# finlaymiller/torch-vae

Hardware: AMD Instinct MI355X
Metric: training samples/sec (VAE step: forward+ELBO+backward+AdamW), synthetic pianoroll (higher is better)
Workload: dtype bf16; 1 GPU; VanillaVAE latent_dim=16, 128x128 synthetic pianoroll, batch 256/GPU (generalised bottleneck 256*(H/16)^2); img_size=128, latent_dim=16, batch_per_gpu=256, global_batch=256, parallelism=dp1, optimizer=AdamW+OneCycle (encoder, decoder groups)

## Files before the change

### include/vae_step.h

```cpp
#ifndef VAE_STEP_H
#define VAE_STEP_H
#include <stdint.h>
#ifdef __cplusplus
extern "C" {
#endif

typedef struct vae_ctx vae_ctx;
typedef void* vae_stream_t;

#define VAE_NUM_PARAMS 40
#define VAE_NUM_BN 8
#define VAE_DTYPE_F32 0
#define VAE_DTYPE_BF16 1
#define VAE_DTYPE_F16 2

const char* vae_last_error(void);
int vae_abi_version(void);

int vae_param_layout(int img_size, int latent_dim, int generalised, int64_t* offsets ,
                     int64_t* sizes , int64_t* total);
int vae_bn_layout(int64_t* offsets , int64_t* channels , int64_t* total);

vae_ctx* vae_create(int img_size, int latent_dim, int max_batch, int dtype, int generalised);
void vae_destroy(vae_ctx* ctx);
// ... 112 lines not shown
                                 int skip_nonfinite, int64_t* step, double* norm_out, int64_t* skipped, void* scratch,
                                 int exchange, float* xhat, float* mu, float* log_var, float* z, float* out3,
                                 vae_stream_t stream);

int vae_synth_pianoroll(float* x, int batch, int img_size, uint64_t seed, vae_stream_t stream);

int vae_expand_stimuli(const void* src, int kind, float* dst, int64_t n_cells, vae_stream_t stream);

int vae_gather_rolls(const void* src, int kind, int64_t n_rolls, int h, int src_w, const int64_t* index, int64_t first,
                     const int32_t* params, uint64_t seed, uint64_t counter0, uint64_t counter_stride, int max_pitch_shift,
                     int max_time_shift, int crop_mode, float scale, float* dst, int batch, int w, vae_stream_t stream);
int vae_augment_params(int32_t* params, int batch, int src_w, int w, uint64_t seed, uint64_t counter0, uint64_t counter_stride,
                       int max_pitch_shift, int max_time_shift, int crop_mode, vae_stream_t stream);

int vae_extract_notes(const float* rolls, int64_t n, int h, int w, float onset_threshold, float sustain_threshold,
                      int min_duration, int max_gap, int32_t* events , float* peaks ,
                      int64_t capacity, int64_t* offsets , uint8_t* cleaned , vae_stream_t stream);

int vae_nearest_rolls(const uint8_t* queries , int n_queries,
                      const uint8_t* rolls   ,   int64_t n_rolls, int h, int w,
                      int max_pitch_shift, int max_time_shift, const int64_t* exclude ,
                      int k, int splits ,
                      int64_t* index , int32_t* distance ,
                      int32_t* shift , int32_t* intersection ,
                      int32_t* query_cells , vae_stream_t stream);

int vae_profile(vae_ctx* ctx, int enable);
int vae_profile_report(vae_ctx* ctx, char* buf, int64_t capacity);
int vae_profile_sequence(vae_ctx* ctx, char* buf, int64_t capacity);
int vae_profile_timeline(vae_ctx* ctx, char* buf, int64_t capacity);
int vae_debug_stamps(vae_ctx* ctx, const char* tag, int epi, long long* out);

int vae_debug_tensor(vae_ctx* ctx, int which, float* out, int64_t capacity, vae_stream_t stream);
int vae_selftest_tr16(vae_stream_t stream);
int vae_set_option(vae_ctx* ctx, const char* name, int value);
int vae_option_info(int index, const char** name, int* default_value);

#ifdef __cplusplus
}
#endif
#endif
```

### torch_vae_amd/_lib.py

```python
from __future__ import annotations

import ctypes as C
import os

_HERE = os.path.dirname(os.path.abspath(__file__))
LIB_PATH = os.environ.get("VAE_STEP_LIB") or os.path.join(_HERE, "lib", "libvae_step_gfx950.so")

NUM_PARAMS = 40
NUM_BN = 8
DTYPE_F32 = 0
DTYPE_BF16 = 1
DTYPE_F16 = 2
RECON_BCE = 0
RECON_MSE = 1
RECON_WBCE = 2
POS_WEIGHT_MAX = 1024.0
KL_PLAIN = 0
KL_FREE_BITS = 1
KL_CAPACITY = 2
KL_TC = 3
TC_MAX_BATCH = 4096
RECON_METRICS_MAX_THRESHOLDS = 8
COMM_ID_BYTES = 128
ROLLS_BYTES, ROLLS_BITS, ROLLS_F32 = 0, 1, 2
# ... 66 lines not shown
    _sig(L.vae_recon_metrics, i32, [p, p, i64, i64, f32p, i32, f32, p, p, p, p, i32, p])
    _sig(L.vae_backward, i32, [p, p, p, p, p, p, p, p, p, p, f32, i32, p])
    _sig(L.vae_backward_part, i32, [p, p, p, p, p, p, p, p, p, p, f32, i32, i32, p])
    _sig(L.vae_encode, i32, [p, p, i32, p, p, p, p, u64, i32, p, p, p, p])
    _sig(L.vae_backward_ex, i32, [p, p, p, p, p, p, p, p, p, p, f32, i32, p, p, p])
    _sig(L.vae_comm_stream, i32, [p, p, C.POINTER(C.c_void_p)])
    _sig(L.vae_comm_unique_id, i32, [p])
    _sig(L.vae_comm_init, i32, [p, i32, i32, p])
    _sig(L.vae_comm_world, i32, [p])
    _sig(L.vae_comm_destroy, i32, [p])
    _sig(L.vae_allreduce_grads, i32, [p, p, i32, i64p, i64p, i32, p])
    _sig(L.vae_broadcast_state, i32, [p, p, p, p, i32, p])
    _sig(L.vae_adamw_step, i32, [p, p, p, p, i32, i64p, i64p, f64p, f64p, f64, f64, f64, f32, i32, p])
    _sig(L.vae_grad_norm, i32, [p, i32, i64p, i64p, f32, p, p, p])
    _sig(L.vae_adamw_step_clipped, i32, [p, p, p, p, i32, i64p, i64p, f64p, f64p, f64, f64, f64, f32, f64, i32, p, p, p, p, p])
    _sig(L.vae_train_step, i32, [p, p, i32, p, p, p, p, p, p, p, u64, f32, i32, i64p, i64p, f64p, f64p, f64, f64, f64,
                                 i32, p, p, p, p, p, p])
    _sig(L.vae_train_step_fused, i32, [p, p, i32, p, p, p, p, p, p, p, u64, f32, i32, i64p, i64p, f64p, f64p, f64, f64, f64, f32,
                                       i32, i32, p, p, p, p, p, p])
    _sig(L.vae_train_step_fused_clipped, i32, [p, p, i32, p, p, p, p, p, p, p, u64, f32, i32, i64p, i64p, f64p, f64p, f64, f64, f64,
                                               f32, f64, i32, p, p, p, p, i32, p, p, p, p, p, p])
    _sig(L.vae_synth_pianoroll, i32, [p, i32, i32, u64, p])
    _sig(L.vae_expand_stimuli, i32, [p, i32, p, i64, p])
    _sig(L.vae_gather_rolls, i32, [p, i32, i64, i32, i32, p, i64, p, u64, u64, u64, i32, i32, i32, f32, p, i32, i32, p])
    _sig(L.vae_augment_params, i32, [p, i32, i32, i32, u64, u64, u64, i32, i32, i32, p])
    _sig(L.vae_extract_notes, i32, [p, i64, i32, i32, f32, f32, i32, i32, p, p, i64, p, p, p])
    _sig(L.vae_nearest_rolls, i32, [p, i32, p, i64, i32, i32, i32, i32, p, i32, i32, p, p, p, p, p, p])
    _sig(L.vae_profile, i32, [p, i32])
    _sig(L.vae_profile_report, i32, [p, C.c_char_p, i64])
    _sig(L.vae_profile_sequence, i32, [p, C.c_char_p, i64])
    _sig(L.vae_profile_timeline, i32, [p, C.c_char_p, i64])
    _sig(L.vae_debug_stamps, i32, [p, C.c_char_p, i32, p])
    _sig(L.vae_debug_tensor, i32, [p, i32, p, i64, p])
    _sig(L.vae_selftest_tr16, i32, [p])
    _sig(L.vae_set_option, i32, [p, C.c_char_p, i32])
    _sig(L.vae_option_info, i32, [i32, C.POINTER(C.c_char_p), C.POINTER(C.c_int)])
    _lib = L
    return L


EXPORTS = [
    "vae_last_error", "vae_abi_version", "vae_param_layout", "vae_bn_layout", "vae_create", "vae_destroy",
    "vae_workspace_bytes", "vae_forward", "vae_decode", "vae_pre_latents", "vae_last_eps", "vae_loss", "vae_loss_deferred", "vae_elbo_generic",
    "vae_set_recon_loss", "vae_set_recon_loss_ex", "vae_elbo_generic_ex", "vae_set_kl_objective", "vae_elbo_generic_kl", "vae_elbo_generic_w", "vae_kl_per_dim", "vae_total_correlation", "vae_last_total_correlation", "vae_log_likelihood", "vae_latent_stats",
    "vae_recon_metrics",
    "vae_backward", "vae_backward_part", "vae_encode", "vae_backward_ex", "vae_comm_stream", "vae_comm_unique_id", "vae_comm_init", "vae_comm_world",
    "vae_comm_destroy", "vae_allreduce_grads", "vae_broadcast_state", "vae_adamw_step", "vae_train_step", "vae_train_step_fused",
    "vae_grad_norm", "vae_adamw_step_clipped", "vae_train_step_fused_clipped", "vae_synth_pianoroll", "vae_expand_stimuli", "vae_profile",
    "vae_profile_report", "vae_profile_sequence", "vae_profile_timeline", "vae_debug_stamps", "vae_debug_tensor",
    "vae_selftest_tr16", "vae_set_option", "vae_option_info", "vae_gather_rolls", "vae_augment_params",
    "vae_extract_notes", "vae_nearest_rolls",
]


def check(rc: int, what: str = ""):
    if rc != 0:
        raise VaeLibError(f"{what}: {lib().vae_last_error().decode()}")


def param_layout(img_size: int, latent_dim: int, generalised: bool):
    offs = (C.c_int64 * NUM_PARAMS)()
    sizes = (C.c_int64 * NUM_PARAMS)()
    total = C.c_int64()
    rc = lib().vae_param_layout(img_size, latent_dim, int(generalised), offs, sizes, C.byref(total))
    if rc != 0:
        raise ValueError(lib().vae_last_error().decode())
    return list(offs), list(sizes), total.value


def bn_layout():
    offs = (C.c_int64 * NUM_BN)()
    ch = (C.c_int64 * NUM_BN)()
    total = C.c_int64()
    check(lib().vae_bn_layout(offs, ch, C.byref(total)), "vae_bn_layout")
    return list(offs), list(ch), total.value


def ptr(t):
    return 0 if t is None else t.data_ptr()
```

### torch_vae_amd/csrc/edge_kernels.cuh

```cuda
#pragma once
#include "common.cuh"

__device__ __forceinline__ float cg_sum(float v) {
#pragma unroll
    for (int o = 4; o < 64; o <<= 1) v += __shfl_xor(v, o, 64);
    return v;
}

template <typename T> __device__ __forceinline__ void load8(const T* p, float* o);
template <> __device__ __forceinline__ void load8<float>(const float* p, float* o) {
    f32x4 a = *reinterpret_cast<const f32x4*>(p), b = *reinterpret_cast<const f32x4*>(p + 4);
#pragma unroll
    for (int i = 0; i < 4; ++i) { o[i] = a[i]; o[4 + i] = b[i]; }
}
template <> __device__ __forceinline__ void load8<bf16>(const bf16* p, float* o) {
    bf16x8 a = *reinterpret_cast<const bf16x8*>(p);
#pragma unroll
    for (int i = 0; i < 8; ++i) o[i] = (float)a[i];
}
template <> __device__ __forceinline__ void load8<f16>(const f16* p, float* o) {
    f16x8 a = *reinterpret_cast<const f16x8*>(p);
#pragma unroll
    for (int i = 0; i < 8; ++i) o[i] = (float)a[i];
}
// ... 864 lines not shown
        const int K = d.k_is_first ? d.A : d.Bc, N = d.k_is_first ? d.Bc : d.A, pairs = d.A * d.Bc;
        for (int pr = blockIdx.x * blockDim.x + threadIdx.x; pr < pairs; pr += gridDim.x * blockDim.x) {
            const int ai = pr / d.Bc, bi = pr - ai * d.Bc;
            const int k = d.k_is_first ? ai : bi, n = d.k_is_first ? bi : ai;
            const float* sp = d.src + (size_t)pr * 9;
            float w[9];
#pragma unroll
            for (int t = 0; t < 9; ++t) w[t] = sp[t];
            const int o = ((k >> 3) * N + n) * 8 + (k & 7), plane = (K >> 3) * N * 8;
#pragma unroll
            for (int t = 0; t < 9; ++t) dst[t * plane + o] = fromfloat<T>(w[t]);
        }
        return;
    }
    for (int i = blockIdx.x * blockDim.x + threadIdx.x; i < total; i += gridDim.x * blockDim.x) {
        if (d.kind == 0) {
        } else if (d.kind == 1) {
            const int e = i & 7; const int r = i >> 3; const int n = r % d.npad; const int fp = (r / d.npad) * 8 + e;
            const int F = 256 * d.s2; const int fr = (fp & 255) * d.s2 + (fp >> 8);
            float v = 0.f;
            if (n < d.L) v = d.src[(long)n * F + fr]; else if (n < 2 * d.L) v = d.src2[(long)(n - d.L) * F + fr];
            dst[i] = fromfloat<T>(v);
        } else if (d.kind == 2) {
            const int e = i & 7; const int r = i >> 3; const int n = r % d.npad; const int fp = (r / d.npad) * 8 + e;
            const int fr = (fp & 255) * d.s2 + (fp >> 8);
            dst[i] = fromfloat<T>(n < d.L ? d.src[(long)fr * d.L + n] : 0.f);
        } else {
            const int t = i / d.A, c = i % d.A;
            reinterpret_cast<float*>(d.dst)[i] = d.src[c * 9 + t];
        }
    }
}

struct AdamGroup { long off, n; float beta1, omb1, decay; float step_size, inv_sqrt_bc2; };
struct AdamArgs {
    float* p; const float* g; float* m; float* v;
    AdamGroup grp[2]; int ngrp;
    float beta2, omb2, eps, grad_scale; int step;
};
template <bool CLIP = false>
__device__ __forceinline__ void adamw_one(float& p, float g, float& m, float& v, const AdamGroup& gr, const AdamArgs& a, float decay,
                                          float coef = 1.f) {
    g *= a.grad_scale;
    if (CLIP) g *= coef;
    p *= decay;
    m = m * gr.beta1 + gr.omb1 * g;
    v = v * a.beta2 + a.omb2 * g * g;
    const float denom = sqrtf(v) * gr.inv_sqrt_bc2 + a.eps;
    p -= gr.step_size * (m / denom);
}
template <bool CLIP = false>
__device__ __forceinline__ void adamw_range(const AdamArgs& a, const AdamGroup& gr, float coef = 1.f) {
    const float decay = gr.decay;
    const long n4 = (gr.off & 3) == 0 ? gr.n >> 2 : 0;
    for (long i = (long)blockIdx.x * blockDim.x + threadIdx.x; i < n4; i += (long)gridDim.x * blockDim.x) {
        const long k = gr.off + 4 * i;
        f32x4 p = *reinterpret_cast<const f32x4*>(a.p + k), m = *reinterpret_cast<const f32x4*>(a.m + k), v = *reinterpret_cast<const f32x4*>(a.v + k);
        const f32x4 g = *reinterpret_cast<const f32x4*>(a.g + k);
#pragma unroll
        for (int e = 0; e < 4; ++e) { float pe = p[e], me = m[e], ve = v[e]; adamw_one<CLIP>(pe, g[e], me, ve, gr, a, decay, coef); p[e] = pe; m[e] = me; v[e] = ve; }
        *reinterpret_cast<f32x4*>(a.p + k) = p; *reinterpret_cast<f32x4*>(a.m + k) = m; *reinterpret_cast<f32x4*>(a.v + k) = v;
    }
    for (long i = 4 * n4 + (long)blockIdx.x * blockDim.x + threadIdx.x; i < gr.n; i += (long)gridDim.x * blockDim.x) {
        const long k = gr.off + i;
        float pe = a.p[k], me = a.m[k], ve = a.v[k];
        adamw_one<CLIP>(pe, a.g[k], me, ve, gr, a, decay, coef);
// ... 43 lines not shown
```

### torch_vae_amd/csrc/vae_api.hip

```cpp
#include <map>
#include <mutex>
#include "vae_ctx.h"
#include "edge_kernels.cuh"
#include "loglik.cuh"
#include "grad_clip.cuh"
#include "total_corr.cuh"

static thread_local std::string g_err;
int vae_set_error(const char* what, const char* why) {
    g_err = std::string(what) + ": " + why;
    return -1;
}

extern "C" const char* vae_last_error(void) { return g_err.c_str(); }
extern "C" int vae_abi_version(void) { return 1; }

static void param_shapes(int H, int L, int gen, int64_t* sizes) {
    const int s = gen ? H / 16 : 2;
    const int64_t F = 256LL * s * s;
    const int enc_ci[4] = {1, 32, 64, 128}, enc_co[4] = {32, 64, 128, 256};
    int k = 0;
    for (int i = 0; i < 4; ++i) { sizes[k++] = 9LL * enc_ci[i] * enc_co[i]; sizes[k++] = enc_co[i]; sizes[k++] = enc_co[i]; sizes[k++] = enc_co[i]; }
    sizes[k++] = L * F; sizes[k++] = L; sizes[k++] = L * F; sizes[k++] = L; sizes[k++] = F * L; sizes[k++] = F;
    const int dec_ci[3] = {256, 128, 64}, dec_co[3] = {128, 64, 32};
// ... 48 lines not shown
    return d;
}

extern "C" void vae_destroy(vae_ctx* c) {
    if (!c) return;
    (void)vae_comm_destroy(c);
    for (void* p : c->allocs) (void)hipFree(p);
    if (c->ll_kb) (void)hipFree(c->ll_kb);
    if (c->n_side_ok) {
        for (int i = 0; i < vae_ctx::NSIDE; ++i) { (void)hipStreamSynchronize(c->side[i]); (void)hipEventDestroy(c->ev_join[i]); }
        (void)hipStreamSynchronize(c->comm);
        for (int i = 0; i < vae_ctx::NFORK; ++i) (void)hipEventDestroy(c->ev_fork[i]);
        (void)hipEventDestroy(c->ev_pack); (void)hipEventDestroy(c->ev_comm);
        if (c->ev_kl) (void)hipEventDestroy(c->ev_kl);
        for (int i = 0; i < vae_ctx::NBUCKET; ++i) (void)hipEventDestroy(c->ev_bucket[i]);
    }
    delete c;
}
extern "C" int64_t vae_workspace_bytes(const vae_ctx* c) { return c ? c->ws_bytes : 0; }

struct OptionDef { const char* name; int& (*ref)(vae_ctx&); int def; int (*norm)(int); };
static int opt_any(int v) { return v; }
static int opt_min1(int v) { return std::max(1, v); }
static int opt_fused_grid(int v) { return std::max(1, std::min(v, 512)); }
static int opt_max1024(int v) { return std::min(v, 1024); }
static int opt_max48(int v) { return std::min(v, 48); }
static int opt_fused_wgrad(int v) { return v == 1 ? 3 : v == 2 ? 1 : v == 3 ? 2 : 0; }
#define OPT(member, def, norm) {#member, [](vae_ctx& c) -> int& { return c.member; }, def, norm}
#define OPT_WK(member, def, norm) {"knob_wgrad_" #member, [](vae_ctx& c) -> int& { return c.wk.member; }, def, norm}
static const OptionDef kOptions[] = {
    OPT(use_tr16, 1, opt_any), OPT(use_mfma_convout, 1, opt_any), OPT(use_pipelined, 1, opt_any), OPT(use_side_stream, 1, opt_any),
    OPT(use_fused_bn, 1, opt_any), OPT(use_fused_convout, 1, opt_any), OPT(use_fused_wgrad, 1, opt_fused_wgrad), OPT(use_recomp_dz, 0, opt_any),
    OPT(use_raw_wgrad, 0, opt_any), OPT(use_deep, 1, opt_any), OPT(use_latent_mfma, 6, opt_any), OPT(use_convout_stream, 1, opt_any),
    OPT(use_dnf_stream, 1, opt_any), OPT(use_upf_stream, 1, opt_any), OPT(use_fc_dgrad8, 1, opt_any), OPT(use_wgrad_split, 1, opt_any),
    OPT(knob_up_per_cu, 2, opt_any), OPT(knob_down_per_cu, 2, opt_min1), OPT(knob_bwd_per_cu, 0, opt_any), OPT(knob_nt_max, 4, opt_any),
    OPT(knob_up_nt_max, 1, opt_min1), OPT(knob_wave_nt_max, 4, opt_any), OPT(knob_lay22_min_nt, 2, opt_any), OPT(knob_lay42, 1, opt_any),
    OPT(knob_down_waves, 8, opt_any), OPT(knob_pipe_max_cout, 256, opt_any), OPT(knob_xcd_map, 1, opt_any), OPT(knob_rev, 4, opt_any),
    OPT(knob_lean, 1, opt_any), OPT(knob_pack_grid, 128, opt_min1), OPT(knob_conv1_grid, 512, opt_any), OPT(knob_fused_grid, 256, opt_fused_grid),
    OPT(knob_convout_grid, 1536, opt_any), OPT(knob_convout_bwd_grid, 1024, opt_any), OPT(knob_convout_step_grid, 1024, opt_min1),
    OPT(knob_convout_bands, 0, opt_any), OPT(knob_wgrad_layer_wgs, 0, opt_any), OPT(knob_skip_wgrad, 0, opt_any), OPT(knob_ablate_b, 0, opt_any),
    OPT(knob_ablate_f, 0, opt_any),
    OPT_WK(tile, 1, opt_any), OPT_WK(wide, 1, opt_any), OPT_WK(mid8, 0, opt_any), OPT_WK(force_simple, 0, opt_any),
    OPT_WK(wgs, 128, opt_max1024), OPT_WK(wide_wgs, 128, opt_max1024), OPT_WK(cap_mb, 48, opt_max48),
};
#undef OPT_WK
#undef OPT
static const OptionDef* find_option(const char* name) {
    for (const OptionDef& o : kOptions) if (name && !strcmp(name, o.name)) return &o;
    return nullptr;
}

extern "C" vae_ctx* vae_create(int H, int L, int maxB, int dtype, int gen) {
    vae_ctx* c = new vae_ctx();
    c->H = H; c->L = L; c->maxB = maxB; c->dtype = dtype; c->gen = gen;
    for (const OptionDef& o : kOptions) o.ref(*c) = o.norm(o.def);
    if (getenv("VAE_NO_SIDE_STREAM")) c->use_side_stream = 0;
    if (vae_param_layout(H, L, gen, c->poff, c->psz, &c->ptotal) != 0) { delete c; return nullptr; }
    if (dtype != VAE_DTYPE_F32 && dtype != VAE_DTYPE_BF16 && dtype != VAE_DTYPE_F16) { vae_set_error("vae_create", "bad dtype"); delete c; return nullptr; }
    if (maxB < 1) { vae_set_error("vae_create", "max_batch < 1"); delete c; return nullptr; }
    vae_bn_layout(c->bnoff, c->bnc, &c->bntotal);
    c->s = gen ? H / 16 : 2; c->s2 = c->s * c->s; c->F = 256LL * c->s2;
    c->npad_fc = (int)align_up(2 * L, 32); c->npad_di = (int)align_up(L, 32);
    c->esz = dtype == VAE_DTYPE_F32 ? 4 : 2;
    const size_t B = maxB;
    const int hs[8] = {H / 2, H / 4, H / 8, H / 16, 2 * c->s, 4 * c->s, 8 * c->s, 16 * c->s};
    size_t nd = 0;
    for (int i = 0; i < 8; ++i) nd += 4 * kBnC[i];
    nd *= STAT_R;
    c->n_dstats = nd + 8 * STAT_R;
    c->dstats = dalloc<double>(c, c->n_dstats);
    bool ok = c->dstats != nullptr;
    double* dp = c->dstats;
    for (int i = 0; i < 8 && ok; ++i) {
        BnLayer& l = c->lay[i];
        l.C = kBnC[i]; l.H = hs[i]; l.W = hs[i];
        l.stat_f = dp; dp += 2 * l.C * STAT_R;
        const size_t n = B * l.H * l.W * l.C;
        l.y = dalloc<char>(c, n * c->esz); l.dz = dalloc<char>(c, n * c->esz); l.block = dalloc<float>(c, LC_ROWS * l.C);
        ok = l.y && l.dz && l.block;
        const int base = i < 4 ? 4 * i : (i < 7 ? 22 + 4 * (i - 4) : 34);
        l.p_convw = base; l.p_convb = base + 1; l.p_gamma = base + 2; l.p_beta = base + 3;
    }
    for (int i = 0; i < 8; ++i) { c->lay[i].stat_b = dp; dp += 2 * kBnC[i] * STAT_R; }
    c->accum = dp;
    if (ok) {
        c->d0 = dalloc<char>(c, B * c->F * c->esz); c->dd0 = dalloc<char>(c, B * c->F * c->esz);
        c->eps = dalloc<float>(c, B * L); c->dlat = dalloc<float>(c, B * 2 * L);
        c->dlogit = dalloc<float>(c, B * H * H); c->dlogit2 = dalloc<float>(c, B * H * H); c->ident = dalloc<float>(c, 3 * 256); c->wout_t = dalloc<float>(c, 288);
        ok = c->d0 && c->dd0 && c->eps && c->dlat && c->dlogit && c->dlogit2 && c->ident && c->wout_t;
    }
    const int ci[8] = {1, 32, 64, 128, 256, 128, 64, 32}, co[8] = {32, 64, 128, 256, 128, 64, 32, 32};
    for (int i = 1; i < 8 && ok; ++i) {
        const size_t n = (size_t)9 * ci[i] * co[i];
        c->wp_fwd[i] = dalloc<char>(c, n * c->esz); c->wp_dg[i] = dalloc<char>(c, n * c->esz);
        ok = c->wp_fwd[i] && c->wp_dg[i];
    }
    if (ok) {
        c->fcpack = dalloc<char>(c, (size_t)c->F * c->npad_fc * c->esz);
        c->dipack = dalloc<char>(c, (size_t)c->F * c->npad_di * c->esz);
        c->d_descs = dalloc<PackDesc>(c, 32);
        ok = c->fcpack && c->dipack && c->d_descs;
    }
    size_t slab = 2048 * 288;
    if (ok) {
        int a, b2, wa, wb;
        for (int wide = 0; wide < 2; ++wide)
            for (int big = 0; big < 2; ++big) {
                if (wide && dtype == VAE_DTYPE_F32) continue;
                for (int i = 1; i < 4; ++i) slab = std::max(slab, wgrad_slab_floats(c->wk, maxB, c->lay[i].H, c->lay[i].W, co[i], ci[i], &a, &b2, &wa, &wb, wide != 0, big != 0));
                for (int i = 4; i < 8; ++i) slab = std::max(slab, wgrad_slab_floats(c->wk, maxB, c->lay[i].H / 2, c->lay[i].W / 2, ci[i], co[i], &a, &b2, &wa, &wb, wide != 0, big != 0));
            }
        const size_t ksteps = c->F / 16;
        slab = std::max(slab, (size_t)std::min<size_t>(ksteps, 512) * maxB * c->npad_fc);
        slab = std::max(slab, (size_t)std::min<size_t>(ksteps, 512) * maxB * c->npad_di);
        slab = std::max(slab, (size_t)8 * (2 * (size_t)L * c->F + c->F));
        c->slab_floats = slab;
        c->slab = dalloc<float>(c, slab);
        ok = c->slab != nullptr;
        for (int i = 0; i < vae_ctx::NSIDE && ok; ++i) { c->side_slab[i] = dalloc<float>(c, slab); ok = c->side_slab[i] != nullptr; }
        if (ok) {
            int prio_least = 0, prio_greatest = 0, side_prio = 0;
            (void)hipDeviceGetStreamPriorityRange(&prio_least, &prio_greatest);
            if (const char* e = getenv("VAE_SIDE_PRIORITY")) side_prio = !strcmp(e, "low") ? prio_least : !strcmp(e, "high") ? prio_greatest : 0;
            DevStreams* ds = device_streams(side_prio);
            ok = ds != nullptr;
            for (int i = 0; i < vae_ctx::NSIDE && ok; ++i) {
                c->side[i] = ds->side[i];
                ok = hipEventCreateWithFlags(&c->ev_join[i], hipEventDisableTiming) == hipSuccess;
            }
            for (int i = 0; i < vae_ctx::NFORK && ok; ++i) ok = hipEventCreateWithFlags(&c->ev_fork[i], hipEventDisableTiming) == hipSuccess;
            if (ok) { c->comm = ds->comm;
                      ok = hipEventCreateWithFlags(&c->ev_pack, hipEventDisableTiming) == hipSuccess &&
                           hipEventCreateWithFlags(&c->ev_comm, hipEventDisableTiming) == hipSuccess;
                      for (int i = 0; i < vae_ctx::NBUCKET && ok; ++i) ok = hipEventCreateWithFlags(&c->ev_bucket[i], hipEventDisableTiming) == hipSuccess; }
// ... 666 lines not shown
    return 0;
}

extern "C" int vae_debug_tensor(vae_ctx* c, int which, float* out, int64_t capacity, vae_stream_t stream) {
    if (!c || !c->fwd) return vae_set_error("vae_debug_tensor", "no forward");
    const void* src; int C, HW;
    if (which == 18) {
        const long n = (long)c->fwd.B * 2 * c->L;
        if (n > capacity) return vae_set_error("vae_debug_tensor", "output too small");
        HIP_CHECK_RET(hipMemcpyAsync(out, c->dlat, (size_t)n * 4, hipMemcpyDeviceToDevice, (hipStream_t)stream));
        return 0;
    }
    if (which == 19) {
        if (c->fwd.kl_kind == VAE_KL_PLAIN || !c->fwd.kl_pending) return vae_set_error("vae_debug_tensor", "the last forward ran with the plain KL objective");
        if (c->L > capacity) return vae_set_error("vae_debug_tensor", "output too small");
        if (join_kl(c, (hipStream_t)stream)) return -1;
        HIP_CHECK_RET(hipMemcpyAsync(out, c->kl_factor(), (size_t)c->L * 4, hipMemcpyDeviceToDevice, (hipStream_t)stream));
        return 0;
    }
    if (which == 20) {
        const long n = (long)c->fwd.B * 2 * c->L;
        if (n > capacity) return vae_set_error("vae_debug_tensor", "output too small");
        if (ensure_tc("vae_debug_tensor", c, (hipStream_t)stream)) return -1;
        HIP_CHECK_RET(hipMemcpyAsync(out, c->tc_grad(), (size_t)n * 4, hipMemcpyDeviceToDevice, (hipStream_t)stream));
        return 0;
    }
    if (which >= 0 && which < 16) { const BnLayer& l = c->lay[which & 7]; src = which < 8 ? l.y : l.dz; C = l.C; HW = l.H * l.W; }
    else if (which == 16 || which == 17) { src = which == 16 ? c->d0 : c->dd0; C = 256; HW = c->s2; }
    else return vae_set_error("vae_debug_tensor", "bad tensor id");
    const long n = (long)c->fwd.B * C * HW;
    if (n > capacity) return vae_set_error("vae_debug_tensor", "output too small");
    return VAE_DISPATCH(c->dtype, debug_tensor_impl, (c, src, out, n, C, HW, (hipStream_t)stream));
}
```

### torch_vae_amd/csrc/vae_ctx.h

```cpp
#pragma once
#include <hip/hip_runtime.h>
#include <stdio.h>
#include <string.h>
#include <math.h>
#include <string>
#include <vector>
#include <algorithm>
#include <map>
#include <mutex>
#include <utility>
#include <type_traits>

#include "../../include/vae_step.h"

int vae_set_error(const char* what, const char* why);

#include "common.cuh"

#define LAUNCH_CHECK(name)                                                        \
    do {                                                                          \
        hipError_t _e = hipGetLastError();                                        \
        if (_e != hipSuccess) return vae_set_error(name, hipGetErrorString(_e)); \
    } while (0)

// ... 37 lines not shown
    if (kept_stream_scratch(bytes, st, &base)) return -1;
    return body(base);
}

static const int kBnC[8] = {32, 64, 128, 256, 128, 64, 32, 32};
static const char* const kLayerTag[8] = {"encoder.0", "encoder.1", "encoder.2", "encoder.3", "decoder.0", "decoder.1", "decoder.2", "final_layer.0"};
static const float kSlope = 0.01f;
static const float kBnEps = 1e-5f;
static const float kBnMom = 0.1f;

static inline int64_t align_up(int64_t v, int64_t a) { return (v + a - 1) / a * a; }
static inline int ilog2(int v) { int l = 0; while ((1 << l) < v) ++l; return l; }

struct Tiling { int lth, ltw, lTB, tiles_x, tiles_y; };
static Tiling make_tiling(int Hs, int Ws, int pixels) {
    const int tw = std::min(Ws, pixels >= 128 ? 16 : 8), th = std::min(Hs, pixels / tw), TB = pixels / (th * tw);
    Tiling t; t.lth = ilog2(th); t.ltw = ilog2(tw); t.lTB = ilog2(TB); t.tiles_x = Ws / tw; t.tiles_y = Hs / th;
    return t;
}

struct BnLayer {
    int C, H, W;
    double* stat_f; double* stat_b; float* block; void* y; void* dz;
    int p_gamma, p_beta, p_convw, p_convb;
    void* act = nullptr; void* dy = nullptr; int act_ok = 0, dy_ok = 0;
};

struct PackDesc {
    const float* src; const float* src2; void* dst;
    int kind;
    int A, Bc, k_is_first, npad, L, s2;
    long n;
};

struct WgradKnobs { int wgs, cap_mb, tile, wide, wide_wgs, small_wgs = 1024, mid8, force_simple; };

struct FwdRecord {
    enum Kind { NONE, FULL, ENCODE, DECODE };
    Kind kind = NONE;
    int B = 0, trained = 0;
    int recon = VAE_RECON_BCE, kl_kind = VAE_KL_PLAIN; double kl_param = 0.0; double recon_param = 0.0;
    int kl_pending = 0;
    int kl_reduced = 0;
    int tc_done = 0;
    const float* x = nullptr; float *xhat = nullptr, *mu = nullptr, *lv = nullptr, *z = nullptr;
    float gmul = 1.f, ginv = 1.f;
    int convout_pending = 0, dlogit_valid = 0; BnFuse pending_f7; float* loss_out3 = nullptr; float loss_kw = 0.f;
    int bwd_dirty = 1;
    int bwd_half_done = 0;
    int walk_dir = 0;
    explicit operator bool() const { return kind != NONE; }
};

struct vae_ctx {
    int H, L, maxB, dtype, gen, s, s2; int64_t F; int npad_fc, npad_di; size_t esz;
    int64_t poff[VAE_NUM_PARAMS], psz[VAE_NUM_PARAMS], ptotal, bnoff[8], bnc[8], bntotal;
    BnLayer lay[8];
    void *d0, *dd0;
    float *eps, *dlat, *dlogit, *dlogit2, *ident, *wout_t;
    void* wp_fwd[8]; void* wp_dg[8];
    void *fcpack, *dipack;
    PackDesc* d_descs; std::vector<PackDesc> h_descs; const float* packed_for = nullptr;
    float* slab; size_t slab_floats;
    static constexpr int NSIDE = 3, NFORK = 16;
    hipStream_t side[NSIDE]; float* side_slab[NSIDE]; hipEvent_t ev_fork[NFORK], ev_join[NSIDE], ev_pack; int side_rr = 0, fork_rr = 0, n_side_ok = 0;
    static constexpr int NBUCKET = 2; hipEvent_t ev_bucket[NBUCKET];
    hipStream_t comm; hipEvent_t ev_comm; int comm_busy = 0;
    void* nccl_comm = nullptr; int comm_rank = 0, comm_world = 0;
    double* dstats; size_t n_dstats; double* accum;
    float* reduce_tmp = nullptr; size_t reduce_tmp_floats = 0; unsigned reduce_slot = 0;
    float* fused_slab[3] = {nullptr, nullptr, nullptr}; size_t fused_slab_floats = 0;
    static constexpr int KL_SIDE = 2;
    void* kl_ws = nullptr; unsigned* kl_tk = nullptr; hipEvent_t ev_kl = nullptr;
    unsigned long long* kl_d() const { return static_cast<unsigned long long*>(kl_ws); }
    double* kl_scal() const { return reinterpret_cast<double*>(kl_d() + L); }
    float* kl_factor() const { return reinterpret_cast<float*>(kl_scal() + 2); }
    const double* kl_shaped() const { return fwd.kl_kind != VAE_KL_PLAIN ? kl_scal() : nullptr; }
    void* tc_ws = nullptr; size_t tc_ws_bytes = 0; int tc_ws_B = 0;
    float* tc_grad() const { return static_cast<float*>(tc_ws); }
    double* ps_part = nullptr; int ps_tb = 0, ps_ntile = 0;
    float* ll_f = nullptr; double* ll_part = nullptr; double* ll_lat = nullptr;
    double* ll_kb = nullptr; size_t ll_kb_n = 0;
    std::vector<void*> allocs; int64_t ws_bytes = 0;
    int use_tr16, use_mfma_convout, use_pipelined, use_side_stream, use_fused_bn, use_fused_convout, use_fused_wgrad, use_recomp_dz, use_raw_wgrad,
        use_deep, use_latent_mfma, use_convout_stream, use_dnf_stream, use_upf_stream, use_fc_dgrad8, use_wgrad_split;
    int knob_up_per_cu, knob_down_per_cu, knob_bwd_per_cu, knob_nt_max, knob_up_nt_max, knob_wave_nt_max, knob_lay22_min_nt, knob_lay42,
        knob_down_waves, knob_pipe_max_cout, knob_xcd_map, knob_rev, knob_lean, knob_pack_grid, knob_conv1_grid, knob_fused_grid,
        knob_convout_grid, knob_convout_bwd_grid, knob_convout_step_grid, knob_convout_bands, knob_wgrad_layer_wgs,
        knob_skip_wgrad, knob_ablate_b, knob_ablate_f;
    WgradKnobs wk;
    int recon = VAE_RECON_BCE, kl_kind = VAE_KL_PLAIN; double kl_param = 0.0; double recon_param = 0.0;
    FwdRecord fwd;
    long long* dbg_buf = nullptr; char dbg_tag[32] = {0}; int dbg_epi = 0;
    int prof = 0; const char* tag = nullptr; struct ProfRec { std::string name; hipEvent_t e0, e1; double bytes, flops; int side; int launches = 1; }; std::vector<ProfRec> prof_recs;
    hipStream_t cur_stream = nullptr; bool cur_stream_set = false;
};

struct ProfScope {
    vae_ctx* c; hipStream_t st; int idx;
    ProfScope(vae_ctx* c_, const char* name, double bytes, double flops, hipStream_t st_) : c(c_), st(st_), idx(-1) {
        if (!c || !c->prof) return;
        vae_ctx::ProfRec r; r.name = std::string(name) + (c->tag ? std::string(" @") + c->tag : std::string()); r.bytes = bytes; r.flops = flops;
        r.side = (c->cur_stream_set && st != c->cur_stream) ? 1 : 0;
        if (hipEventCreate(&r.e0) != hipSuccess || hipEventCreate(&r.e1) != hipSuccess) return;
        (void)hipEventRecord(r.e0, st);
        c->prof_recs.push_back(r); idx = (int)c->prof_recs.size() - 1;
    }
    ~ProfScope() { if (idx >= 0) (void)hipEventRecord(c->prof_recs[idx].e1, st); }
    ProfScope(const ProfScope&) = delete;
    ProfScope& operator=(const ProfScope&) = delete;
};

static inline size_t wgrad_slab_floats(const WgradKnobs& k, int B, int Hs, int Ws, int CA, int CB, int* nsplit_out, int* tps_out, int* WA_out, int* WB_out,
                                       bool wide_ok = false, bool big = false) {
    int WA, WB;
    if (wide_ok && k.wide && CA >= 128 && k.tile == 1) { WA = 4; WB = 1; }
    else if (CA >= 64 && CB >= 64 && k.tile == 0) { WA = 2; WB = 2; } else if (CA >= 64 && k.tile <= 1) { WA = 2; WB = 1; } else { WA = 1; WB = 1; }
    Tiling t = make_tiling(Hs, Ws, WG_KP);
// ... 85 lines not shown
```

### torch_vae_amd/csrc/vae_impl.cuh

```cuda
#pragma once
#include "vae_ctx.h"
#include "conv_mfma.cuh"
#include "conv_pipe.cuh"
#include "edge_kernels.cuh"
#include "conv_fused.cuh"
#include "conv_deep.cuh"
#include "latent_mfma.cuh"
#include "convout_stream.cuh"
#include "wgrad_split.cuh"
#include "upfinal_stream.cuh"
#include "dnfirst_stream.cuh"
#include "grad_paths.cuh"

template <typename F> static int pick_recon(vae_ctx* c, F&& f) {
    return pick_const<VAE_RECON_BCE, VAE_RECON_MSE, VAE_RECON_WBCE>("reconstruction term", c->fwd.recon, f);
}
template <typename F> static int pick_recon_per_sample(vae_ctx* c, F&& f) {
    return pick_const<VAE_RECON_BCE, VAE_RECON_MSE>("reconstruction term", c->fwd.recon == VAE_RECON_WBCE ? VAE_RECON_BCE : c->fwd.recon, f);
}

static int stream_bands(int B, int rows, int max_bands, int min_rows, int rows_per_tick, int fixed_ticks) {
    const int ncu = 256;
    long best = -1; int nb = 1;
    for (int cand = 1; cand <= max_bands && rows / cand >= min_rows; cand *= 2) {
// ... 258 lines not shown
static int launch_dense(vae_ctx* c, DenseArgs<T> a, int* nsplit_out, hipStream_t st) {
    const int nb = a.Npad / 32, NT = nb % 4 == 0 ? 4 : (nb % 2 == 0 ? 2 : 1);
    if (a.Npad % 32) return vae_set_error("dense", "Npad must be a multiple of 32");
    const int mt = (a.M + 127) / 128, ntile = a.Npad / (32 * NT), ksteps = a.K / 16;
    int nsplit = std::max(1, std::min(ksteps, 512 / std::max(1, mt * ntile)));
    a.ksteps_per_split = (ksteps + nsplit - 1) / nsplit;
    nsplit = (ksteps + a.ksteps_per_split - 1) / a.ksteps_per_split;
    if ((size_t)nsplit * a.M * a.Npad > c->slab_floats) return vae_set_error("dense", "slab too small");
    a.slab = c->slab;
    dim3 grid(mt, nsplit, ntile);
    *nsplit_out = nsplit;
    ProfScope ps(c, "dense(fc / decoder_input dgrad)", sizeof(T) * ((double)a.M * a.K + (double)a.K * a.Npad), 2.0 * a.M * a.K * a.Npad, st);
    return pick_const<1, 2, 4>("dense_kernel", NT, [&](auto N) { return launch("dense_kernel", dense_kernel<T, decltype(N)::value>, grid, dim3(256), 0, st, a); });
}
template <typename T>
int pack_weights(vae_ctx* c, const float* params, hipStream_t st) {
    std::vector<PackDesc>& d = c->h_descs;
    if (c->packed_for != params || d.empty()) {
        d.clear();
        const int ci[8] = {1, 32, 64, 128, 256, 128, 64, 32}, co[8] = {32, 64, 128, 256, 128, 64, 32, 32};
        for (int i = 1; i < 8; ++i) {
            const bool conv = i < 4;
            PackDesc p; memset(&p, 0, sizeof(p));
            p.src = params + c->poff[c->lay[i].p_convw]; p.kind = 0; p.n = 9L * ci[i] * co[i];
            p.A = conv ? co[i] : ci[i]; p.Bc = conv ? ci[i] : co[i];
            p.dst = c->wp_fwd[i]; p.k_is_first = conv ? 0 : 1; d.push_back(p);
            p.dst = c->wp_dg[i]; p.k_is_first = conv ? 1 : 0; d.push_back(p);
        }
        PackDesc p; memset(&p, 0, sizeof(p));
        p.kind = 1; p.src = params + c->poff[16]; p.src2 = params + c->poff[18]; p.dst = c->fcpack; p.npad = c->npad_fc; p.L = c->L; p.s2 = c->s2; p.n = c->F * c->npad_fc; d.push_back(p);
        p.kind = 2; p.src = params + c->poff[20]; p.src2 = nullptr; p.dst = c->dipack; p.npad = c->npad_di; p.n = c->F * c->npad_di; d.push_back(p);
        p.kind = 3; p.src = params + c->poff[38]; p.dst = c->wout_t; p.A = 32; p.n = 288; d.push_back(p);
        HIP_CHECK_RET(hipMemcpyAsync(c->d_descs, d.data(), d.size() * sizeof(PackDesc), hipMemcpyHostToDevice, st));
        c->packed_for = params;
    }
    ProfScope ps(c, "pack_weights", 0, 0, st);
    return launch("pack_kernel", pack_kernel<T>, dim3((unsigned)c->knob_pack_grid, (unsigned)d.size()), dim3(256), 0, st, c->d_descs);
}

static BnFuse make_fuse_fwd(vae_ctx* c, int i, const float* params, float* bn_running, int64_t* nbt) {
    const BnLayer& l = c->lay[i];
    BnFuse f; memset(&f, 0, sizeof(f));
    f.stat = l.stat_f; f.gamma = params + c->poff[l.p_gamma]; f.beta = params + c->poff[l.p_beta]; f.block = l.block;
    f.running_mean = bn_running ? bn_running + c->bnoff[i] : nullptr; f.running_var = bn_running ? bn_running + c->bnoff[i] + l.C : nullptr;
    f.nbt = nbt ? reinterpret_cast<long long*>(nbt) + i : nullptr;
    f.C = l.C; f.count = (double)c->fwd.B * l.H * l.W; f.inv_count = 1.0 / f.count; f.eps = kBnEps; f.momentum = kBnMom; f.update_running = bn_running != nullptr;
    f.mode = BNF_FWD;
    return f;
}
static BnFuse make_fuse_bwd(vae_ctx* c, int i, const float* params, float* grads) {
    const BnLayer& l = c->lay[i];
    BnFuse f; memset(&f, 0, sizeof(f));
    f.stat = l.stat_b; f.gamma = params + c->poff[l.p_gamma]; f.block = l.block;
    f.dgamma = grads + c->poff[l.p_gamma]; f.dbeta = grads + c->poff[l.p_beta]; f.dconv_bias = grads + c->poff[l.p_convb];
    f.C = l.C; f.count = (double)c->fwd.B * l.H * l.W; f.inv_count = 1.0 / f.count; f.mode = BNF_BWD; f.ginv = c->fwd.ginv;
    return f;
}
static int bn_finalize_now(vae_ctx* c, const BnFuse& f, hipStream_t st) {
    ProfScope ps(c, f.mode == BNF_FWD ? "bn_fwd_finalize" : "bn_bwd_finalize", 0, 0, st);
    return launch("bn_finalize_kernel", bn_finalize_kernel, dim3(1), dim3(256), 0, st, f);
}
static int bn_bwd_for(vae_ctx* c, int i, bool consumer_fuses, const float* params, float* grads, BnFuse* out, hipStream_t st) {
    *out = make_fuse_bwd(c, i, params, grads);
    if (consumer_fuses && c->use_fused_bn && c->fwd.trained) return 0;
    if (c->fwd.trained) { if (bn_finalize_now(c, *out, st)) return -1; }
    else {
        ProfScope ps(c, "bn_eval_bwd_finalize", 0, 0, st);
        if (launch("bn_eval_bwd_kernel", bn_eval_bwd_kernel, dim3(1), dim3(256), 0, st, *out)) return -1;
    }
// ... 597 lines not shown
```

Measured before the change: 238,200 samples/s.

## Pack weights with an LDS-tiled transpose kernel over a precomputed tile list

After: 240,200 samples/s, median of 6. Within noise of the previous version (+0.8%).

```diff
diff --git a/include/vae_step.h b/include/vae_step.h
--- a/include/vae_step.h
+++ b/include/vae_step.h
@@ -168,6 +168,7 @@
 int vae_debug_stamps(vae_ctx* ctx, const char* tag, int epi, long long* out);
 
 int vae_debug_tensor(vae_ctx* ctx, int which, float* out, int64_t capacity, vae_stream_t stream);
+int vae_debug_packed(vae_ctx* ctx, int which, void* out, int64_t capacity, int64_t* bytes, int fill);
 int vae_selftest_tr16(vae_stream_t stream);
 int vae_set_option(vae_ctx* ctx, const char* name, int value);
 int vae_option_info(int index, const char** name, int* default_value);
diff --git a/torch_vae_amd/_lib.py b/torch_vae_amd/_lib.py
--- a/torch_vae_amd/_lib.py
+++ b/torch_vae_amd/_lib.py
@@ -122,6 +122,7 @@
     _sig(L.vae_profile_timeline, i32, [p, C.c_char_p, i64])
     _sig(L.vae_debug_stamps, i32, [p, C.c_char_p, i32, p])
     _sig(L.vae_debug_tensor, i32, [p, i32, p, i64, p])
+    _sig(L.vae_debug_packed, i32, [p, i32, p, i64, i64p, i32])
     _sig(L.vae_selftest_tr16, i32, [p])
     _sig(L.vae_set_option, i32, [p, C.c_char_p, i32])
     _sig(L.vae_option_info, i32, [i32, C.POINTER(C.c_char_p), C.POINTER(C.c_int)])
@@ -137,7 +138,7 @@
     "vae_backward", "vae_backward_part", "vae_encode", "vae_backward_ex", "vae_comm_stream", "vae_comm_unique_id", "vae_comm_init", "vae_comm_world",
     "vae_comm_destroy", "vae_allreduce_grads", "vae_broadcast_state", "vae_adamw_step", "vae_train_step", "vae_train_step_fused",
     "vae_grad_norm", "vae_adamw_step_clipped", "vae_train_step_fused_clipped", "vae_synth_pianoroll", "vae_expand_stimuli", "vae_profile",
-    "vae_profile_report", "vae_profile_sequence", "vae_profile_timeline", "vae_debug_stamps", "vae_debug_tensor",
+    "vae_profile_report", "vae_profile_sequence", "vae_profile_timeline", "vae_debug_stamps", "vae_debug_tensor", "vae_debug_packed",
     "vae_selftest_tr16", "vae_set_option", "vae_option_info", "vae_gather_rolls", "vae_augment_params",
     "vae_extract_notes", "vae_nearest_rolls",
 ]
diff --git a/torch_vae_amd/csrc/edge_kernels.cuh b/torch_vae_amd/csrc/edge_kernels.cuh
--- a/torch_vae_amd/csrc/edge_kernels.cuh
+++ b/torch_vae_amd/csrc/edge_kernels.cuh
@@ -920,6 +920,103 @@
     }
 }
 
+static constexpr int PK_CROW = PK_TB * 9 + 4;
+static constexpr int PK_FROW = PK_NB * 8 + 4;
+static constexpr int PK_LDS = PK_PB * PK_FROW > PK_TA * PK_CROW ? PK_PB * PK_FROW : PK_TA * PK_CROW;
+template <typename T>
+__device__ __forceinline__ void pack_store8(T* dst, const float (&v)[8]) {
+    constexpr int N = Vec16<T>::N;
+#pragma unroll
+    for (int h = 0; h < 8 / N; ++h) {
+        Vec16<T> o;
+#pragma unroll
+        for (int e = 0; e < N; ++e) o.set(e, v[h * N + e]);
+        *reinterpret_cast<Vec16<T>*>(dst + h * N) = o;
+    }
+}
+template <typename T>
+__global__ void __launch_bounds__(256) pack_tiled_kernel(const PackTensor* __restrict__ tens, const PackTile* __restrict__ tiles) {
+    __shared__ __attribute__((aligned(16))) float s[PK_LDS];
+    const PackTile tl = tiles[blockIdx.x];
+    const PackTensor d = tens[tl.tensor];
+    const int tid = threadIdx.x;
+    if (d.kind == 0) {
+        const int a0 = tl.i0, b0 = tl.i1;
+        constexpr int RUN4 = PK_TB * 9 / 4;
+        for (int i = tid; i < PK_TA * RUN4; i += 256) {
+            const int ai = i / RUN4, q = i - ai * RUN4;
+            *reinterpret_cast<f32x4*>(&s[ai * PK_CROW + q * 4]) = *reinterpret_cast<const f32x4*>(d.src + ((size_t)(a0 + ai) * d.Bc + b0) * 9 + q * 4);
+        }
+        __syncthreads();
+        T* const dA = reinterpret_cast<T*>(d.dst); T* const dB = reinterpret_cast<T*>(d.dst2);
+        const size_t plane = (size_t)d.A * d.Bc;
+        for (int i = tid; i < 9 * PK_TB; i += 256) {
+            const int t = i / PK_TB, bi = i % PK_TB;
+            float v[8];
+#pragma unroll
+            for (int e = 0; e < 8; ++e) v[e] = s[e * PK_CROW + bi * 9 + t];
+            pack_store8<T>(dA + t * plane + ((size_t)(a0 >> 3) * d.Bc + b0 + bi) * 8, v);
+        }
+        for (int i = tid; i < 9 * (PK_TB / 8) * PK_TA; i += 256) {
+            const int t = i / (PK_TB / 8 * PK_TA), g = (i / PK_TA) % (PK_TB / 8), ai = i % PK_TA;
+            float v[8];
+#pragma unroll
+            for (int e = 0; e < 8; ++e) v[e] = s[ai * PK_CROW + (g * 8 + e) * 9 + t];
+            pack_store8<T>(dB + t * plane + ((size_t)((b0 >> 3) + g) * d.A + a0 + ai) * 8, v);
+        }
+        return;
+    }
+    if (d.kind == 3) {
+        if (tid < 72) *reinterpret_cast<f32x4*>(&s[tid * 4]) = *reinterpret_cast<const f32x4*>(d.src + tid * 4);
+        __syncthreads();
+        if (tid < 72) {
+            const int t = tid >> 3, c = (tid & 7) * 4;
+            f32x4 o;
+#pragma unroll
+            for (int e = 0; e < 4; ++e) o[e] = s[(c + e) * 9 + t];
+            *reinterpret_cast<f32x4*>(reinterpret_cast<float*>(d.dst) + tid * 4) = o;
+        }
+        return;
+    }
+    const int c8 = tl.i0, p0 = tl.i1, pb = d.pb, lpb = 31 - __clz(pb);
+    const size_t F = (size_t)256 * d.s2;
+    T* const dst = reinterpret_cast<T*>(d.dst);
+    for (int n0 = 0; n0 < d.npad; n0 += PK_NB) {
+        if (n0) __syncthreads();
+        if (d.kind == 1) {
+            for (int i = tid; i < PK_NB * 8 * (pb >> 2); i += 256) {
+                const int p4 = i & ((pb >> 2) - 1), e = (i >> (lpb - 2)) & 7, nn = i >> (lpb + 1), n = n0 + nn;
+                f32x4 w = {0.f, 0.f, 0.f, 0.f};
+                if (n < d.nreal) w = *reinterpret_cast<const f32x4*>((n < d.L ? d.src + (size_t)n * F : d.src2 + (size_t)(n - d.L) * F) + (size_t)(c8 * 8 + e) * d.s2 + p0 + p4 * 4);
+#pragma unroll
+                for (int j = 0; j < 4; ++j) s[(p4 * 4 + j) * PK_FROW + nn * 8 + e] = w[j];
+            }
+        } else if ((d.L & 3) == 0) {
+            for (int i = tid; i < 8 * pb * (PK_NB / 4); i += 256) {
+                const int n4 = i & (PK_NB / 4 - 1), pp = (i >> 3) & (pb - 1), e = i >> (lpb + 3), n = n0 + n4 * 4;
+                f32x4 w = {0.f, 0.f, 0.f, 0.f};
+                if (n < d.nreal) w = *reinterpret_cast<const f32x4*>(d.src + ((size_t)(c8 * 8 + e) * d.s2 + p0 + pp) * d.L + n);
+#pragma unroll
+                for (int j = 0; j < 4; ++j) s[pp * PK_FROW + (n4 * 4 + j) * 8 + e] = w[j];
+            }
+        } else {
+            for (int i = tid; i < 8 * pb * PK_NB; i += 256) {
+                const int nn = i & (PK_NB - 1), pp = (i >> 5) & (pb - 1), e = i >> (lpb + 5), n = n0 + nn;
+                s[pp * PK_FROW + nn * 8 + e] = n < d.nreal ? d.src[((size_t)(c8 * 8 + e) * d.s2 + p0 + pp) * d.L + n] : 0.f;
+            }
+        }
+        __syncthreads();
+        for (int i = tid; i < pb * PK_NB; i += 256) {
+            const int nn = i & (PK_NB - 1), pp = i >> 5;
+            float v[8];
+            const f32x4 lo = *reinterpret_cast<const f32x4*>(&s[pp * PK_FROW + nn * 8]), hi = *reinterpret_cast<const f32x4*>(&s[pp * PK_FROW + nn * 8 + 4]);
+#pragma unroll
+            for (int e = 0; e < 4; ++e) { v[e] = lo[e]; v[4 + e] = hi[e]; }
+            pack_store8<T>(dst + (((size_t)(p0 + pp) * 32 + c8) * d.npad + n0 + nn) * 8, v);
+        }
+    }
+}
+
 struct AdamGroup { long off, n; float beta1, omb1, decay; float step_size, inv_sqrt_bc2; };
 struct AdamArgs {
     float* p; const float* g; float* m; float* v;
diff --git a/torch_vae_amd/csrc/vae_api.hip b/torch_vae_amd/csrc/vae_api.hip
--- a/torch_vae_amd/csrc/vae_api.hip
+++ b/torch_vae_amd/csrc/vae_api.hip
@@ -104,7 +104,7 @@
     OPT(use_tr16, 1, opt_any), OPT(use_mfma_convout, 1, opt_any), OPT(use_pipelined, 1, opt_any), OPT(use_side_stream, 1, opt_any),
     OPT(use_fused_bn, 1, opt_any), OPT(use_fused_convout, 1, opt_any), OPT(use_fused_wgrad, 1, opt_fused_wgrad), OPT(use_recomp_dz, 0, opt_any),
     OPT(use_raw_wgrad, 0, opt_any), OPT(use_deep, 1, opt_any), OPT(use_latent_mfma, 6, opt_any), OPT(use_convout_stream, 1, opt_any),
-    OPT(use_dnf_stream, 1, opt_any), OPT(use_upf_stream, 1, opt_any), OPT(use_fc_dgrad8, 1, opt_any), OPT(use_wgrad_split, 1, opt_any),
+    OPT(use_dnf_stream, 1, opt_any), OPT(use_upf_stream, 1, opt_any), OPT(use_fc_dgrad8, 1, opt_any), OPT(use_wgrad_split, 1, opt_any), OPT(use_pack_tiled, 1, opt_any),
     OPT(knob_up_per_cu, 2, opt_any), OPT(knob_down_per_cu, 2, opt_min1), OPT(knob_bwd_per_cu, 0, opt_any), OPT(knob_nt_max, 4, opt_any),
     OPT(knob_up_nt_max, 1, opt_min1), OPT(knob_wave_nt_max, 4, opt_any), OPT(knob_lay22_min_nt, 2, opt_any), OPT(knob_lay42, 1, opt_any),
     OPT(knob_down_waves, 8, opt_any), OPT(knob_pipe_max_cout, 256, opt_any), OPT(knob_xcd_map, 1, opt_any), OPT(knob_rev, 4, opt_any),
@@ -171,7 +171,8 @@
         c->fcpack = dalloc<char>(c, (size_t)c->F * c->npad_fc * c->esz);
         c->dipack = dalloc<char>(c, (size_t)c->F * c->npad_di * c->esz);
         c->d_descs = dalloc<PackDesc>(c, 32);
-        ok = c->fcpack && c->dipack && c->d_descs;
+        c->d_ptens = dalloc<PackTensor>(c, 16); c->d_ptiles = dalloc<PackTile>(c, pack_tile_count(c->s2));
+        ok = c->fcpack && c->dipack && c->d_descs && c->d_ptens && c->d_ptiles;
     }
     size_t slab = 2048 * 288;
     if (ok) {
@@ -904,3 +905,21 @@
     if (n > capacity) return vae_set_error("vae_debug_tensor", "output too small");
     return VAE_DISPATCH(c->dtype, debug_tensor_impl, (c, src, out, n, C, HW, (hipStream_t)stream));
 }
+
+extern "C" int vae_debug_packed(vae_ctx* c, int which, void* out, int64_t capacity, int64_t* bytes, int fill) {
+    if (!c) return vae_set_error("vae_debug_packed", "null ctx");
+    if (!c->packed_for) return vae_set_error("vae_debug_packed", "no weights packed yet");
+    void* src; int64_t n;
+    if (which >= 0 && which < 14) { const int i = 1 + which % 7; src = which < 7 ? c->wp_fwd[i] : c->wp_dg[i]; n = 9LL * kConvCi[i] * kConvCo[i] * (int64_t)c->esz; }
+    else if (which == 14) { src = c->fcpack; n = c->F * c->npad_fc * (int64_t)c->esz; }
+    else if (which == 15) { src = c->dipack; n = c->F * c->npad_di * (int64_t)c->esz; }
+    else if (which == 16) { src = c->wout_t; n = 288 * 4; }
+    else return vae_set_error("vae_debug_packed", "bad image id");
+    if (bytes) *bytes = n;
+    if (out && n > capacity) return vae_set_error("vae_debug_packed", "output too small");
+    if (!out && fill < 0) return 0;
+    HIP_CHECK_RET(hipDeviceSynchronize());
+    if (out) HIP_CHECK_RET(hipMemcpy(out, src, (size_t)n, hipMemcpyDefault));
+    if (fill >= 0) { HIP_CHECK_RET(hipMemset(src, fill & 255, (size_t)n)); HIP_CHECK_RET(hipDeviceSynchronize()); }
+    return 0;
+}
diff --git a/torch_vae_amd/csrc/vae_ctx.h b/torch_vae_amd/csrc/vae_ctx.h
--- a/torch_vae_amd/csrc/vae_ctx.h
+++ b/torch_vae_amd/csrc/vae_ctx.h
@@ -93,6 +93,23 @@
     int A, Bc, k_is_first, npad, L, s2;
     long n;
 };
+
+static constexpr int PK_TA = 8, PK_TB = 32;
+static constexpr int PK_PB = 16, PK_NB = 32;
+struct PackTensor {
+    const float* src; const float* src2; void* dst; void* dst2;
+    int kind;
+    int A, Bc;
+    int npad, nreal, L, s2, pb;
+};
+struct PackTile { int tensor, i0, i1; };
+static constexpr int kConvCi[8] = {1, 32, 64, 128, 256, 128, 64, 32}, kConvCo[8] = {32, 64, 128, 256, 128, 64, 32, 32};
+static inline int pack_pb(int s2) { return std::min(s2, PK_PB); }
+static inline int pack_tile_count(int s2) {
+    int n = 1;
+    for (int i = 1; i < 8; ++i) n += kConvCi[i] * kConvCo[i] / (PK_TA * PK_TB);
+    return n + 2 * 32 * (s2 / pack_pb(s2));
+}
 
 struct WgradKnobs { int wgs, cap_mb, tile, wide, wide_wgs, small_wgs = 1024, mid8, force_simple; };
 
@@ -122,6 +139,7 @@
     void* wp_fwd[8]; void* wp_dg[8];
     void *fcpack, *dipack;
     PackDesc* d_descs; std::vector<PackDesc> h_descs; const float* packed_for = nullptr;
+    PackTensor* d_ptens; PackTile* d_ptiles; std::vector<PackTensor> h_ptens; std::vector<PackTile> h_ptiles;
     float* slab; size_t slab_floats;
     static constexpr int NSIDE = 3, NFORK = 16;
     hipStream_t side[NSIDE]; float* side_slab[NSIDE]; hipEvent_t ev_fork[NFORK], ev_join[NSIDE], ev_pack; int side_rr = 0, fork_rr = 0, n_side_ok = 0;
@@ -144,7 +162,7 @@
     double* ll_kb = nullptr; size_t ll_kb_n = 0;
     std::vector<void*> allocs; int64_t ws_bytes = 0;
     int use_tr16, use_mfma_convout, use_pipelined, use_side_stream, use_fused_bn, use_fused_convout, use_fused_wgrad, use_recomp_dz, use_raw_wgrad,
-        use_deep, use_latent_mfma, use_convout_stream, use_dnf_stream, use_upf_stream, use_fc_dgrad8, use_wgrad_split;
+        use_deep, use_latent_mfma, use_convout_stream, use_dnf_stream, use_upf_stream, use_fc_dgrad8, use_wgrad_split, use_pack_tiled;
     int knob_up_per_cu, knob_down_per_cu, knob_bwd_per_cu, knob_nt_max, knob_up_nt_max, knob_wave_nt_max, knob_lay22_min_nt, knob_lay42,
         knob_down_waves, knob_pipe_max_cout, knob_xcd_map, knob_rev, knob_lean, knob_pack_grid, knob_conv1_grid, knob_fused_grid,
         knob_convout_grid, knob_convout_bwd_grid, knob_convout_step_grid, knob_convout_bands, knob_wgrad_layer_wgs,
diff --git a/torch_vae_amd/csrc/vae_impl.cuh b/torch_vae_amd/csrc/vae_impl.cuh
--- a/torch_vae_amd/csrc/vae_impl.cuh
+++ b/torch_vae_amd/csrc/vae_impl.cuh
@@ -314,9 +314,40 @@
         p.kind = 2; p.src = params + c->poff[20]; p.src2 = nullptr; p.dst = c->dipack; p.npad = c->npad_di; p.n = c->F * c->npad_di; d.push_back(p);
         p.kind = 3; p.src = params + c->poff[38]; p.dst = c->wout_t; p.A = 32; p.n = 288; d.push_back(p);
         HIP_CHECK_RET(hipMemcpyAsync(c->d_descs, d.data(), d.size() * sizeof(PackDesc), hipMemcpyHostToDevice, st));
+        std::vector<PackTensor>& pt = c->h_ptens; std::vector<PackTile>& tl = c->h_ptiles;
+        pt.clear(); tl.clear();
+        for (int i = 1; i < 8; ++i) {
+            const bool conv = i < 4;
+            PackTensor t; memset(&t, 0, sizeof(t));
+            t.src = params + c->poff[c->lay[i].p_convw]; t.kind = 0;
+            t.A = conv ? kConvCo[i] : kConvCi[i]; t.Bc = conv ? kConvCi[i] : kConvCo[i];
+            t.dst = conv ? c->wp_dg[i] : c->wp_fwd[i]; t.dst2 = conv ? c->wp_fwd[i] : c->wp_dg[i];
+            for (int a0 = 0; a0 < t.A; a0 += PK_TA)
+                for (int b0 = 0; b0 < t.Bc; b0 += PK_TB) tl.push_back(PackTile{(int)pt.size(), a0, b0});
+            pt.push_back(t);
+        }
+        for (int kind = 1; kind <= 2; ++kind) {
+            PackTensor t; memset(&t, 0, sizeof(t));
+            t.kind = kind; t.L = c->L; t.s2 = c->s2; t.pb = pack_pb(c->s2);
+            if (kind == 1) { t.src = params + c->poff[16]; t.src2 = params + c->poff[18]; t.dst = c->fcpack; t.npad = c->npad_fc; t.nreal = 2 * c->L; }
+            else { t.src = params + c->poff[20]; t.dst = c->dipack; t.npad = c->npad_di; t.nreal = c->L; }
+            for (int c8 = 0; c8 < 32; ++c8)
+                for (int p0 = 0; p0 < c->s2; p0 += t.pb) tl.push_back(PackTile{(int)pt.size(), c8, p0});
+            pt.push_back(t);
+        }
+        {
+            PackTensor t; memset(&t, 0, sizeof(t));
+            t.kind = 3; t.src = params + c->poff[38]; t.dst = c->wout_t;
+            tl.push_back(PackTile{(int)pt.size(), 0, 0}); pt.push_back(t);
+        }
+        if ((int)tl.size() != pack_tile_count(c->s2) || pt.size() > 16) return vae_set_error("pack_weights", "work list does not match its allocation");
+        HIP_CHECK_RET(hipMemcpyAsync(c->d_ptens, pt.data(), pt.size() * sizeof(PackTensor), hipMemcpyHostToDevice, st));
+        HIP_CHECK_RET(hipMemcpyAsync(c->d_ptiles, tl.data(), tl.size() * sizeof(PackTile), hipMemcpyHostToDevice, st));
         c->packed_for = params;
     }
     ProfScope ps(c, "pack_weights", 0, 0, st);
+    if (c->use_pack_tiled && !(reinterpret_cast<uintptr_t>(params) & 15))
+        return launch("pack_tiled_kernel", pack_tiled_kernel<T>, dim3((unsigned)c->h_ptiles.size()), dim3(256), 0, st, c->d_ptens, c->d_ptiles);
     return launch("pack_kernel", pack_kernel<T>, dim3((unsigned)c->knob_pack_grid, (unsigned)d.size()), dim3(256), 0, st, c->d_descs);
 }
 
```
